# leaner-forever/SEGS-SLAM

Hardware: AMD Instinct MI355X
Metric: mapper train-iters/sec (fwd+bwd raster) (higher is better)
Workload: dtype f32; 1 GPU; 1080p_3m: 3000000 Gaussians, 1920x1080, 1 keyframe per GPU, fwd+bwd raster; P=3000000, P_visible=2096178, num_rendered=10472370, instances_binned=7913347, instances_live=6766534, width=1920, height=1080, parallelism=keyframe-dp1, forward=resident (no host sync), hipgraph=off

## Files before the change

include/segs_raster.h:

```cpp
#ifndef SEGS_RASTER_H_
#define SEGS_RASTER_H_

#include <stddef.h>
#include <stdint.h>

#ifdef __cplusplus
extern "C" {
#endif

#define SEGS_OK 0
#define SEGS_ERR_INVALID_ARGUMENT (-1)
#define SEGS_ERR_UNSUPPORTED (-2)
#define SEGS_ERR_ALLOC (-3)

typedef char* (*segs_alloc_fn)(void* ctx, size_t bytes);

const char* segs_last_error(void);

#define SEGS_RASTER_SKIP_NONPOSITIVE_OPACITY 1u
#define SEGS_RASTER_KEEP_DEAD_INSTANCES 2u
#define SEGS_RASTER_GATHER_TILES_TOUCHED 4u
#define SEGS_RASTER_TEST_NARROW_PACK 8u
#define SEGS_RASTER_UNFUSED_BINNING 16u
#define SEGS_RASTER_TIGHT_BINNING 32u
#define SEGS_RASTER_MFMA_MOMENTS 64u
#define SEGS_RASTER_NO_WRITTEN_BYTES 128u
uint32_t segs_raster_set_flags(uint32_t flags);

uint32_t* segs_raster_set_status_mirror(uint32_t* host_mapped_status);

size_t segs_geometry_bytes(int P);
size_t segs_image_bytes(int width, int height);
size_t segs_binning_bytes(int num_rendered);

int segs_rasterize_forward(segs_alloc_fn geometry_alloc, void* geometry_ctx,
                           segs_alloc_fn binning_alloc, void* binning_ctx,
                           segs_alloc_fn image_alloc, void* image_ctx,
                           int P, int D, int M,
                           const float* background, int width, int height,
                           const float* means3D, const float* shs, const float* colors_precomp,
                           const float* opacities, const float* scales, float scale_modifier,
                           const float* rotations, const float* cov3D_precomp,
                           const float* viewmatrix, const float* projmatrix, const float* cam_pos,
                           float tan_fovx, float tan_fovy, int prefiltered,
                           float* out_color, int* radii, void* stream, int* num_rendered);

int segs_rasterize_backward(int P, int D, int M, int R,
                            const float* background, int width, int height,
                            const float* means3D, const float* shs, const float* colors_precomp,
                            const float* scales, float scale_modifier, const float* rotations,
                            const float* cov3D_precomp, const float* viewmatrix, const float* projmatrix,
                            const float* campos, float tan_fovx, float tan_fovy, const int* radii,
                            char* geom_buffer, char* binning_buffer, char* image_buffer,
                            const float* dL_dpix, float* dL_dmean2D, float* dL_dconic, float* dL_dopacity,
                            float* dL_dcolor, float* dL_dmean3D, float* dL_dcov3D, float* dL_dsh,
                            float* dL_dscale, float* dL_drot, void* stream);

int segs_visible_filter(int P, int M, int width, int height, const float* means3D, const float* scales,
                        float scale_modifier, const float* rotations, const float* cov3D_precomp,
                        const float* viewmatrix, const float* projmatrix, float tan_fovx, float tan_fovy,
                        int prefiltered, int* radii, void* stream);

int segs_visible_filter_log_scales(int P, int width, int height, const float* means3D, const float* scaling_log, int stride,
                                   const float* rotations, const float* viewmatrix, const float* projmatrix, float tan_fovx,
                                   float tan_fovy, int* radii, void* stream);

int segs_mark_visible(int P, const float* means3D, const float* viewmatrix, const float* projmatrix,
                      uint8_t* present, void* stream);

int segs_project2_image(int P, int D, int M, int width, int height, const float* means3D, const float* shs,
                        const float* colors_precomp, const float* opacities, const float* scales,
                        float scale_modifier, const float* rotations, const float* cov3D_precomp,
                        const float* viewmatrix, const float* projmatrix, const float* cam_pos,
                        float tan_fovx, float tan_fovy, int prefiltered, float* out_color, float* points_image,
                        int* radii, void* stream);

int segs_debug_unpack_geometry(const char* geom_buffer, int P, const int* radii, float* means2D ,
                               float* conic_opacity , float* depths , uint32_t* tiles_touched ,
                               uint32_t* point_offsets , float* rgb , void* stream);
// ... 147 lines not shown
```

segs-slam_amd/csrc/capi.hip:

```cpp
#include <hip/hip_runtime.h>
#include <cstdio>
#include <cstdlib>
#include <algorithm>
#include <cstring>
#include <string>
#include <vector>
#include "../../include/segs_raster.h"
#include "gs_layout.h"
#include "kernels.h"
#include "capi_args.h"

using namespace segs;

namespace {
thread_local std::string g_err;
}
int segs::set_error(int code, const char* what) {
  g_err = what;
  return code;
}
int segs::set_hip_error(hipError_t e, const char* where) {
  g_err = std::string(where) + ": " + hipGetErrorString(e);
  return (int)e > 0 ? (int)e : 1;
}
// ... 238 lines not shown
  PROF(K_RENDER_FWD);
  if (dout && (dout->depth || dout->alpha))
    render_fwd_depth_kernel<<<V.tiles, 256, 0, st>>>(S.ranges(), S.point_list(), V.width, V.height, S.G.rec(), background, S.final_T(),
                                                     S.n_contrib(), out_color, dout->depth, dout->alpha);
  else
    render_fwd_kernel<<<V.tiles, 256, 0, st>>>(S.ranges(), S.point_list(), V.width, V.height, S.G.rec(), background, S.final_T(), S.n_contrib(),
                                               out_color);
  LAUNCH_TRY("render_fwd_kernel");
  return SEGS_OK;
}

int launch_render_bwd(const Scratch& S, const View& V, const float* background, const float* dL_dpix, const segs_depth_grads* dgrad,
                      uint8_t* written, hipStream_t st) {
  PROF(K_RENDER_BWD);
  const uint32_t grid = (V.tiles + 7) / 8 * 32;
  if (dgrad && (dgrad->dL_ddepth || dgrad->dL_dalpha)) {
    render_bwd_depth_kernel<<<grid, 64, 0, st>>>(S.ranges(), S.point_list(), V.width, V.height, S.G.rec(), background, S.final_T(),
                                                 S.n_contrib(), dL_dpix, S.G.gacc(), V.tiles, dgrad->dL_ddepth, dgrad->dL_dalpha, written);
    LAUNCH_TRY("render_bwd_depth_kernel");
    return SEGS_OK;
  }
  static const bool mfma_env = [] { const char* e = getenv("SEGS_RENDER_BWD_MFMA"); return e && e[0] == '1'; }();
  ((mfma_env || (g_flags & SEGS_RASTER_MFMA_MOMENTS)) ? render_bwd_mfma_kernel : render_bwd_kernel)<<<grid, 64, 0, st>>>(
      S.ranges(), S.point_list(), V.width, V.height, S.G.rec(), background, S.final_T(), S.n_contrib(), dL_dpix, S.G.gacc(), V.tiles, written);
  LAUNCH_TRY("render_bwd_kernel");
  return SEGS_OK;
}

int camera_grads_begin(const segs_camera_grads* cam, const float* shs, bool empty, hipStream_t st, bool* live) {
  *live = false;
  if (!cam) return SEGS_OK;
  if (!cam->dL_dviewmatrix || !cam->dL_dprojmatrix || !cam->temp) return fail(SEGS_ERR_INVALID_ARGUMENT, "segs_camera_grads: null field");
  if (shs) return fail(SEGS_ERR_INVALID_ARGUMENT, "camera gradients need colors_precomp: the SH colours depend on campos, which they do not cover");
  if (empty) {
    HIP_TRY(hipMemsetAsync(cam->dL_dviewmatrix, 0, 16 * sizeof(float), st));
    HIP_TRY(hipMemsetAsync(cam->dL_dprojmatrix, 0, 16 * sizeof(float), st));
    return SEGS_OK;
  }
  *live = true;
  return SEGS_OK;
}
float* camera_partials(const segs_camera_grads* cam) { return (float*)align_ptr(cam->temp); }
int camera_grads_finish(const segs_camera_grads* cam, int nblocks, hipStream_t st) {
  camera_grad_reduce_kernel<<<1, 960, 0, st>>>(camera_partials(cam), nblocks, cam->dL_dviewmatrix, cam->dL_dprojmatrix);
  LAUNCH_TRY("camera_grad_reduce_kernel");
  return SEGS_OK;
}

int launch_preprocess_bwd(const Gaussians& g, const View& V, const int* radii, const GradOutputs& o, const PerGaussianBwd& m, hipStream_t st) {
  const bool depth = m.depth || m.dz_in;
  auto* const kernel = m.cam ? (depth ? preprocess_bwd_kernel<true, true> : preprocess_bwd_kernel<false, true>)
                             : (depth ? preprocess_bwd_kernel<true, false> : preprocess_bwd_kernel<false, false>);
  const int nblocks = (g.P + 255) / 256;
  kernel<<<nblocks, 256, 0, st>>>(g.P, g.means3D, radii, g.kernel_scales(), g.rotations, g.scale_modifier, g.cov3D_precomp, V.viewmatrix,
                                  V.projmatrix, V.focal_x, V.focal_y, V.tan_fovx, V.tan_fovy, m.gacc, (float)V.width, (float)V.height,
                                  o.dL_dmean2D, o.dL_dconic, o.dL_dopacity, o.dL_dcolor, o.dL_dmean3D, o.dL_dcov3D, o.dL_dscale, o.dL_drot,
                                  m.clean_gacc ? 1 : 0, m.dz_in, m.cam ? camera_partials(m.cam) : nullptr, m.written);
  LAUNCH_TRY("preprocess_bwd_kernel");
  return m.cam ? camera_grads_finish(m.cam, nblocks, st) : SEGS_OK;
}

int rasterize_forward(const Allocators& A, const Gaussians& g, const View& V, const float* background, float* out_color, int* radii,
                      const segs_depth_outputs* dout, hipStream_t st, int* num_rendered) {
  const int P = g.P;
  if (!A.geometry_alloc || !A.binning_alloc || !A.image_alloc) return fail(SEGS_ERR_INVALID_ARGUMENT, "null allocator callback");
  if (P < 0 || V.width <= 0 || V.height <= 0) return fail(SEGS_ERR_INVALID_ARGUMENT, "bad P / image size");
  if (P > MAX_GAUSSIANS) return fail(SEGS_ERR_INVALID_ARGUMENT, "P exceeds 2^28 Gaussians (sort values carry a 4-bit quadrant mask)");
  if (!background || !out_color || !V.viewmatrix || !V.projmatrix || !num_rendered) return fail(SEGS_ERR_INVALID_ARGUMENT, "null required pointer");
  if (P > 0 && (!g.means3D || !g.opacities)) return fail(SEGS_ERR_INVALID_ARGUMENT, "null means3D/opacities");
  if (P > 0)
    if (int rc = check_colour_and_shape(g, V)) return rc;
  if (int rc = check_tile_grid(V)) return rc;

  Scratch S{};
  char* geom_raw = A.geometry_alloc(A.geometry_ctx, geom_layout(P).total);
  S.IL = image_layout(V.width, V.height);
  char* img_raw = A.image_alloc(A.image_ctx, S.IL.total);
  if (!geom_raw || !img_raw) return fail(SEGS_ERR_ALLOC, "allocator callback returned null");
  S.G = geom_at(geom_raw, P);
  S.img = align_ptr(img_raw);
  const Geom& G = S.G;
  if (!radii) radii = G.radii_internal();

  int R = 0;
  uint32_t hdr[3] = {0u, 0u, 0u};
  const bool tight = (g_flags & SEGS_RASTER_TIGHT_BINNING) != 0u;
  bool fast_keys = tight;
  if (P > 0) {
    K1Targets k1;
    k1.extra_flags = tight ? PREPROCESS_TIGHT_RECT : 0u;
    if (fast_keys) { k1.depth_keys = (uint32_t*)G.bin(); k1.ranges = S.ranges(); }
    int rc = run_preprocess(G, g, V, radii, k1, st);
    if (rc) return rc;
    { PROF(K_SCAN);
    scan_block_sums_kernel<<<1, 1024, 0, st>>>(G.block_sums(), G.L.nblocks, G.block_sums() + (G.L.nblocks + 1), G.num_rendered());
    }
    LAUNCH_TRY("scan_block_sums_kernel");
    HIP_TRY(hipMemcpyAsync(hdr, G.num_rendered(), sizeof(hdr), hipMemcpyDeviceToHost, st));
    HIP_TRY(hipStreamSynchronize(st));
    R = (int)hdr[0];
    if (R < 0) return fail(SEGS_ERR_INVALID_ARGUMENT, "num_rendered overflows int32");
    if (fast_keys && R > 0 && (hdr[2] - DEPTH_KEY_MIN) >= ((1u << DEPTH_KEY_BITS) - 1u)) {
      fast_keys = false;
      K1Targets exact;
      exact.extra_flags = PREPROCESS_TIGHT_RECT;
      rc = run_preprocess(G, g, V, radii, exact, st);
// ... 26 lines not shown
  if (B.geom_rows > MAX_GAUSSIANS) return fail(SEGS_ERR_INVALID_ARGUMENT, "P exceeds 2^28 Gaussians");
  if (!B.geom_buffer || !B.binning_buffer || !B.image_buffer || !status || !others_present) return fail(SEGS_ERR_INVALID_ARGUMENT, "null required pointer");
  if (k1)
    if (int rc = check_colour_and_shape(*k1, V)) return rc;
  if (int rc = check_tile_grid(V)) return rc;
  *S = carve(B, P, V, status);
  return SEGS_OK;
}

int rasterize_forward_resident(const ScratchBuffers& B, int P, const Gaussians* k1, const View& V, const float* background, float* out_color,
                               int* radii, uint32_t* status, const segs_depth_outputs* dout, hipStream_t st) {
  Scratch S{};
  const bool others_present = background && out_color && (!k1 || (V.viewmatrix && V.projmatrix && k1->means3D && k1->opacities));
  if (int rc = open_resident(B, P, V, status, others_present, k1, &S)) return rc;
  const DepthSortInput keys = resident_depth_sort_input(S.bin, S.GS);
  if (k1) {
    K1Targets t;
    t.depth_keys = keys.keys; t.depth_vals = keys.vals; t.ranges = S.ranges();
    t.extra_flags = resident_k1_flags(); t.depth_overflow = status + 2;
    if (int rc = run_preprocess(S.G, *k1, V, radii ? radii : S.G.radii_internal(), t, st)) return rc;
  }
  if (int rc = run_binning(S, V, BinningMode::resident_keys(keys.keys, drop_dead_instances()), st)) return rc;
  return launch_render_fwd(S, V, background, out_color, dout, st);
}

int rasterize_backward(const Gaussians& g, const View& V, const ScratchBuffers& B, const BackwardInputs& in, const GradOutputs& o,
                       GaccCleaning cleaning, hipStream_t st) {
  const int P = g.P, R = B.capacity;
  const bool self_clean = cleaning == SELF_CLEAN;
  if (P < 0 || R < 0 || V.width <= 0 || V.height <= 0) return fail(SEGS_ERR_INVALID_ARGUMENT, "bad sizes");
  if (B.geom_rows < P) return fail(SEGS_ERR_INVALID_ARGUMENT, "geom_rows must be >= P");
  bool cam_live = false;
  if (int rc = camera_grads_begin(in.cam, g.shs, P == 0 || R == 0, st, &cam_live)) return rc;
  if (P == 0) return SEGS_OK;
  if (g.shs && (!V.cam_pos || !o.dL_dsh || g.M <= 0)) return fail(SEGS_ERR_INVALID_ARGUMENT, "SH path needs campos, dL_dsh and M > 0");
  if (!B.geom_buffer || !B.binning_buffer || !B.image_buffer || !in.dL_dpix || !in.background || !g.means3D || !V.viewmatrix || !V.projmatrix)
    return fail(SEGS_ERR_INVALID_ARGUMENT, "null required pointer");
  if (!o.dL_dmean2D || !o.dL_dopacity || !o.dL_dcolor || !o.dL_dmean3D || (g.cov3D_precomp && !o.dL_dcov3D))
    return fail(SEGS_ERR_INVALID_ARGUMENT, "null gradient output");
  if (!g.cov3D_precomp && (!g.scales || !g.rotations || !o.dL_dscale || !o.dL_drot))
    return fail(SEGS_ERR_INVALID_ARGUMENT, "need scales+rotations (+ their gradient outputs) or cov3D_precomp");
  uint32_t* const no_status = nullptr;
  const Scratch S = carve(B, P, V, no_status);
  const Geom& G = S.G;
  const int* radii = in.radii ? in.radii : G.radii_internal();

  if (!self_clean) { PROF(K_MEMSET);
  HIP_TRY(hipMemsetAsync(G.gacc(), 0, (size_t)P * GACC_DWORDS * 4, st));
  }
  PerGaussianBwd m;
  m.gacc = G.gacc(); m.depth = in.dgrad && in.dgrad->dL_ddepth; m.clean_gacc = self_clean;
  if (cam_live) m.cam = in.cam;
  m.written = (self_clean && !(g_flags & SEGS_RASTER_NO_WRITTEN_BYTES)) ? G.written() : nullptr;
  if (R > 0)
    if (int rc = launch_render_bwd(S, V, in.background, in.dL_dpix, in.dgrad, m.written, st)) return rc;
  { PROF(K_PREPROCESS_BWD);
  if (int rc = launch_preprocess_bwd(g, V, radii, o, m, st)) return rc;
  }
  if (g.shs) {
    sh_backward_kernel<<<G.L.nblocks, 256, 0, st>>>(P, g.means3D, radii, g.shs, g.D, g.M, V.cam_pos, G.clamped(), o.dL_dcolor, o.dL_dmean3D, o.dL_dsh);
    LAUNCH_TRY("sh_backward_kernel");
  }
  return SEGS_OK;
}

int visible_filter(const Gaussians& g, const View& V, int log_scale_stride, int* radii, hipStream_t st) {
  if (g.P < 0 || V.width <= 0 || V.height <= 0) return fail(SEGS_ERR_INVALID_ARGUMENT, "bad sizes");
  if (g.P == 0) return SEGS_OK;
  if (!g.means3D || !V.viewmatrix || !V.projmatrix || !radii) return fail(SEGS_ERR_INVALID_ARGUMENT, "null required pointer");
  if (!g.cov3D_precomp && (!g.scales || !g.rotations)) return fail(SEGS_ERR_INVALID_ARGUMENT, "need scales+rotations or cov3D_precomp");
  visible_filter_kernel<<<(g.P + 255) / 256, 256, 0, st>>>(g.P, g.means3D, g.kernel_scales(), g.scale_modifier, g.rotations, g.cov3D_precomp,
                                                           V.viewmatrix, V.projmatrix, V.width, V.height, V.tan_fovx, V.tan_fovy, V.focal_x,
                                                           V.focal_y, V.gx, V.gy, radii, log_scale_stride);
  LAUNCH_TRY("visible_filter_kernel");
  return SEGS_OK;
}

int debug_preprocess_backward(const Gaussians& g, const View& V, const int* radii, const GradOutputs& o, const float* dL_dz,
                              const segs_camera_grads* cam, hipStream_t st) {
  bool cam_live = false;
  if (int rc = camera_grads_begin(cam, g.shs, g.P <= 0, st, &cam_live)) return rc;
  if (g.P <= 0) return SEGS_OK;
  if (!g.means3D || !radii || !V.viewmatrix || !V.projmatrix || !o.dL_dmean2D || !o.dL_dconic || !o.dL_dmean3D || !o.dL_dcov3D)
    return fail(SEGS_ERR_INVALID_ARGUMENT, "null pointer");
  PerGaussianBwd m;
  if (cam_live) { m.dz_in = dL_dz; m.cam = cam; }
  return launch_preprocess_bwd(g, V, radii, o, m, st);
}

}

extern "C" {

const char* segs_last_error(void) { return g_err.c_str(); }

uint32_t* segs_raster_set_status_mirror(uint32_t* host_mapped_status) {
  uint32_t* old = g_status_mirror;
  g_status_mirror = host_mapped_status;
  return old;
}

uint32_t segs_raster_set_flags(uint32_t flags) {
  const uint32_t old = g_flags;
  g_flags = flags;
  return old;
}
// ... 395 lines not shown
```

segs-slam_amd/csrc/capi_args.h:

```cpp
#pragma once
#include <hip/hip_runtime.h>
#include <cstdint>
#include "../../include/segs_raster.h"
#include "gs_layout.h"
#include "kernels.h"

namespace segs {

struct Gaussians {
  int P; const float *means3D, *scales; float scale_modifier; const float *rotations, *cov3D_precomp;
  int D, M; const float *shs, *colors_precomp, *opacities;
  const float* kernel_scales() const { return cov3D_precomp ? nullptr : scales; }
};

struct View {
  int width, height; const float *viewmatrix, *projmatrix, *cam_pos; float tan_fovx, tan_fovy;
  uint32_t gx, gy, tiles; float focal_x, focal_y;
};
inline View image_view(int width, int height) {
  View v{};
  v.width = width; v.height = height;
  v.gx = (width + TILE_X - 1) / TILE_X; v.gy = (height + TILE_Y - 1) / TILE_Y; v.tiles = v.gx * v.gy;
  return v;
}
// ... 54 lines not shown
  ImageLayout IL;
  BinningLayout BL;
  GaussSortLayout GS;
  uint32_t* status;
  uint2* ranges() const { return (uint2*)(img + IL.ranges); }
  const uint32_t* point_list() const { return (const uint32_t*)(bin + BL.vals[0]); }
  float* final_T() const { return (float*)(img + IL.final_T); }
  uint32_t* n_contrib() const { return (uint32_t*)(img + IL.n_contrib); }
};
inline Scratch carve(const ScratchBuffers& B, int P, const View& V, uint32_t* status) {
  return Scratch{geom_at(B.geom_buffer, P, B.geom_rows), align_ptr(B.image_buffer), align_ptr(B.binning_buffer), image_layout(V.width, V.height),
                 binning_layout(B.capacity), gauss_sort_layout(B.capacity, P), status};
}

struct DepthSortInput { uint32_t *keys, *vals; };
inline DepthSortInput depth_sort_input(char* bin, const GaussSortLayout& GS, int dbits, int digit_bits) {
  const int side = sort_first_side(dbits, digit_bits);
  return DepthSortInput{(uint32_t*)(bin + GS.base + GS.inner.keys[side]), (uint32_t*)(bin + GS.base + GS.inner.vals[side])};
}

struct BinningMode {
  uint32_t dmin; int dbits; uint32_t dcull;
  int digit_bits;
  const uint32_t* k1_keys;
  bool drop_dead;
  static constexpr int RESIDENT_DIGIT_BITS = 9;
  static BinningMode resident_keys(const uint32_t* k1_keys, bool drop_dead) {
    return BinningMode{DEPTH_KEY_MIN, DEPTH_KEY_BITS, 0xFFFFFFFFu, RESIDENT_DIGIT_BITS, k1_keys, drop_dead};
  }
  static BinningMode exact_range(uint32_t max_not_depth, uint32_t max_depth, bool drop_dead) {
    const uint32_t dmin = ~max_not_depth, dspan = max_depth - dmin + 1u;
    int dbits = 1;
    while (dbits < 32 && (dspan >> dbits) != 0u) dbits++;
    const bool nine = (dbits + 8) / 9 < (dbits + 7) / 8;
    return BinningMode{dmin, dbits, dmin + dspan, nine ? 9 : 8, nullptr, drop_dead};
  }
};
inline DepthSortInput resident_depth_sort_input(char* bin, const GaussSortLayout& GS) { return depth_sort_input(bin, GS, DEPTH_KEY_BITS, BinningMode::RESIDENT_DIGIT_BITS); }

struct K1Targets {
  uint32_t *depth_keys = nullptr, *depth_vals = nullptr;
  uint2* ranges = nullptr;
  uint32_t extra_flags = 0u;
  uint32_t* depth_overflow = nullptr;
};

struct PerGaussianBwd {
  float* gacc = nullptr;
  bool depth = false;
  bool clean_gacc = false;
  const float* dz_in = nullptr;
  const segs_camera_grads* cam = nullptr;
  uint8_t* written = nullptr;
};

struct Allocators { segs_alloc_fn geometry_alloc; void* geometry_ctx; segs_alloc_fn binning_alloc; void* binning_ctx; segs_alloc_fn image_alloc; void* image_ctx; };

enum GaccCleaning { MEMSET_PER_CALL, SELF_CLEAN };
struct BackwardInputs { const float* background; const int* radii; const float* dL_dpix; const segs_depth_grads* dgrad; const segs_camera_grads* cam; };

constexpr const Gaussians* K1_RAN_AT_PRODUCER = nullptr;
constexpr const segs_depth_outputs* NO_DEPTH_OUTPUTS = nullptr;
constexpr const segs_depth_grads* NO_DEPTH_GRADS = nullptr;
constexpr const segs_camera_grads* NO_CAMERA_GRADS = nullptr;
constexpr const float *NO_CAM_POS = nullptr, *NO_DL_DZ = nullptr;
constexpr int* NO_RADII = nullptr;

}
```

segs-slam_amd/csrc/kernels.h:

```cpp
#pragma once
#include <hip/hip_runtime.h>
#include <cstdint>
#include "gs_layout.h"

namespace segs {

int set_error(int code, const char* what);
int set_hip_error(hipError_t e, const char* where);


__global__ void preprocess_fwd_kernel(
    int P, const float* __restrict__ means3D, const float* __restrict__ scales, float mod,
    const float* __restrict__ rotations, const float* __restrict__ opacities, const float* __restrict__ colors,
    const float* __restrict__ cov3D_precomp, const float* __restrict__ viewmatrix, const float* __restrict__ projmatrix,
    int W, int H, float tan_fovx, float tan_fovy, float focal_x, float focal_y, uint32_t gx, uint32_t gy,
    int* __restrict__ radii, float* __restrict__ rec, BinInfo* __restrict__ bin, uint32_t* __restrict__ block_sums,
    uint32_t* __restrict__ depth_range, const float* __restrict__ shs, int D, int M, const float* __restrict__ cam_pos,
    uint32_t* __restrict__ clamped, uint32_t flags, uint32_t* __restrict__ depth_keys, uint32_t* __restrict__ depth_vals,
    uint2* __restrict__ ranges, int num_tiles, uint32_t* __restrict__ depth_overflow, uint32_t* __restrict__ touched_dense);
constexpr uint32_t DEPTH_KEY_MIN = 0x3E4CCCCDu;
constexpr int DEPTH_KEY_BITS = 27;

__global__ void visible_filter_kernel(
    int P, const float* __restrict__ means3D, const float* __restrict__ scales, float mod,
    const float* __restrict__ rotations, const float* __restrict__ cov3D_precomp,
    const float* __restrict__ viewmatrix, const float* __restrict__ projmatrix, int W, int H,
    float tan_fovx, float tan_fovy, float focal_x, float focal_y, uint32_t gx, uint32_t gy, int* __restrict__ radii,
    int log_scale_stride);

__global__ void mark_visible_kernel(int P, const float* __restrict__ means3D, const float* __restrict__ viewmatrix,
                                    uint8_t* __restrict__ present);

constexpr int CAM_SUMS = 24;
template <bool DEPTH, bool CAM>
__global__ void preprocess_bwd_kernel(
    int P, const float* __restrict__ means3D, const int* __restrict__ radii, const float* __restrict__ scales,
    const float* __restrict__ rotations, float mod, const float* __restrict__ cov3D_precomp,
    const float* __restrict__ view, const float* __restrict__ proj, float h_x, float h_y, float tan_fovx, float tan_fovy,
    float* __restrict__ gacc, float img_w, float img_h,
    float* __restrict__ dL_dmean2D, float* __restrict__ dL_dconic,
    float* __restrict__ dL_dopacity, float* __restrict__ dL_dcolor, float* __restrict__ dL_dmean3D,
    float* __restrict__ dL_dcov3D, float* __restrict__ dL_dscale, float* __restrict__ dL_drot, int clean_gacc,
    const float* __restrict__ dz_in, float* __restrict__ cam_partials, uint8_t* __restrict__ written);
__global__ void camera_grad_reduce_kernel(const float* __restrict__ partials, int nblocks, float* __restrict__ dL_dview,
                                          float* __restrict__ dL_dproj);
__global__ void sh_backward_kernel(int P, const float* __restrict__ means3D, const int* __restrict__ radii,
                                   const float* __restrict__ shs, int D, int M, const float* __restrict__ cam_pos,
                                   const uint32_t* __restrict__ clamped, const float* __restrict__ dL_dcolor,
                                   float* __restrict__ dL_dmean3D, float* __restrict__ dL_dsh);

__global__ void scan_block_sums_kernel(uint32_t* __restrict__ block_sums, int nblocks, const uint32_t* __restrict__ depth_range,
                                       uint32_t* __restrict__ total);
__global__ void ordered_offsets_kernel(int P, const uint32_t* __restrict__ block_sums, uint32_t* __restrict__ incl,
                                       uint32_t* __restrict__ total_out, const uint32_t* __restrict__ ng_dev,
                                       uint32_t* __restrict__ first_owner, uint32_t owner_entries);
__global__ void duplicate_with_keys_kernel(int P, int R, const float* __restrict__ rec,
                                           const uint32_t* __restrict__ order, const uint32_t* __restrict__ incl,
                                           uint32_t* __restrict__ keys, uint32_t* __restrict__ vals, uint32_t gx,
                                           const uint32_t* __restrict__ n_dev, int mark_dead, const uint32_t* __restrict__ ng_dev,
                                           const uint32_t* __restrict__ first_owner);
constexpr uint32_t RANGE_EMPTY_START = 0xFFFFFFFFu;
__global__ void normalize_ranges_kernel(int num_tiles, uint2* __restrict__ ranges);
constexpr uint32_t PREPROCESS_TIGHT_RECT = 0x80000000u;
constexpr uint32_t DEAD_KEY = 0xFFFFFFFFu;
template <typename K, int BITS>
__global__ void radix_count_kernel(const K* __restrict__ keys, int n, int shift, uint32_t dmin, int dbits,
                                   uint32_t* __restrict__ tile_prefix, uint32_t* __restrict__ chunk_hist, int nblocks, int nchunks,
                                   const uint32_t* __restrict__ n_dev, int drop_dead, int chunk_tiles, int nbits);
__global__ void radix_scan_kernel(uint32_t* __restrict__ block_hist, int nblocks, uint32_t* __restrict__ digit_totals);
template <typename K, int BITS, bool AUX>
__global__ void radix_scatter_kernel(const K* __restrict__ keys_in, const uint32_t* __restrict__ vals_in,
                                     K* __restrict__ keys_out, uint32_t* __restrict__ vals_out, int n, int shift,
                                     uint32_t dmin, int dbits, const uint32_t* __restrict__ tile_prefix, const uint32_t* __restrict__ chunk_prefix,
                                     const uint32_t* __restrict__ digit_totals, int nblocks, int nchunks,
                                     const uint32_t* __restrict__ n_dev, int drop_dead, uint32_t* __restrict__ n_live_out,
                                     const uint32_t* __restrict__ aux_in, uint32_t* __restrict__ aux_out, int nbits, int chunk_tiles, int pack_shift,
                                     uint2* __restrict__ ranges_out, uint32_t* __restrict__ status, uint32_t* __restrict__ status_mirror,
                                     int write_keys);
__global__ void identify_tile_ranges_kernel(int L, const uint32_t* __restrict__ keys, uint2* __restrict__ ranges,
                                            const uint32_t* __restrict__ n_dev, uint32_t* __restrict__ status,
                                            uint32_t* __restrict__ status_mirror, const uint32_t* __restrict__ n_live);

__global__ void render_fwd_kernel(const uint2* __restrict__ ranges, const uint32_t* __restrict__ point_list, int W, int H,
                                  const float* __restrict__ rec, const float* __restrict__ bg,
                                  float* __restrict__ final_T, uint32_t* __restrict__ n_contrib, float* __restrict__ out_color);
__global__ void render_bwd_kernel(const uint2* __restrict__ ranges, const uint32_t* __restrict__ point_list, int W, int H,
                                  const float* __restrict__ rec, const float* __restrict__ bg,
                                  const float* __restrict__ final_T, const uint32_t* __restrict__ n_contrib,
                                  const float* __restrict__ dL_dpix, float* __restrict__ gacc, uint32_t num_tiles,
                                  uint8_t* __restrict__ written);
__global__ void render_bwd_mfma_kernel(const uint2* __restrict__ ranges, const uint32_t* __restrict__ point_list, int W, int H,
                                       const float* __restrict__ rec, const float* __restrict__ bg,
                                       const float* __restrict__ final_T, const uint32_t* __restrict__ n_contrib,
                                       const float* __restrict__ dL_dpix, float* __restrict__ gacc, uint32_t num_tiles,
                                       uint8_t* __restrict__ written);
__global__ void render_fwd_depth_kernel(const uint2* __restrict__ ranges, const uint32_t* __restrict__ point_list, int W, int H,
// ... 27 lines not shown
```

segs-slam_amd/csrc/preprocess.hip:

```cpp
#include <hip/hip_runtime.h>
#include <cstdint>
#include "gs_layout.h"
#include "kernels.h"
#include "project_gaussian.h"
#include "sh_color.h"

#pragma clang fp contract(off)

namespace segs {

__device__ __forceinline__ float3 load_row3(const float* __restrict__ a, int P, float* lds ) {
  const int tid = threadIdx.x;
  const size_t base = (size_t)blockIdx.x * 768;
  const size_t lim = (size_t)P * 3;
#pragma unroll
  for (int k = 0; k < 3; k++) {
    const size_t i = base + k * 256 + tid;
    lds[k * 256 + tid] = i < lim ? a[i] : 0.f;
  }
  __syncthreads();
  float3 v = make_float3(lds[3 * tid], lds[3 * tid + 1], lds[3 * tid + 2]);
  __syncthreads();
  return v;
}
// ... 381 lines not shown
      for (int kk = 0; kk < 3; kk++) {
        float ds = 0.f;
#pragma unroll
        for (int i = 0; i < 3; i++) {
          const float dLik = 2.f * (M2[0][i] * DU[0][kk] + M2[1][i] * DU[1][kk]);
          ds += R[i][kk] * dLik;
          GR[i][kk] = dLik * s3[kk];
        }
        out_scale[kk] = ds;
      }
      const float r = q.x, x = q.y, y = q.z, z = q.w;
      out_rot[0] = 2.f * (z * (GR[1][0] - GR[0][1]) + y * (GR[0][2] - GR[2][0]) + x * (GR[2][1] - GR[1][2]));
      out_rot[1] = 2.f * (y * (GR[0][1] + GR[1][0]) + z * (GR[0][2] + GR[2][0]) + r * (GR[2][1] - GR[1][2])) - 4.f * x * (GR[1][1] + GR[2][2]);
      out_rot[2] = 2.f * (x * (GR[0][1] + GR[1][0]) + r * (GR[0][2] - GR[2][0]) + z * (GR[1][2] + GR[2][1])) - 4.f * y * (GR[0][0] + GR[2][2]);
      out_rot[3] = 2.f * (r * (GR[1][0] - GR[0][1]) + x * (GR[0][2] + GR[2][0]) + y * (GR[1][2] + GR[2][1])) - 4.f * z * (GR[0][0] + GR[1][1]);
    }
  }
  if constexpr (CAM) {
    const int v = threadIdx.x >> 5, l = threadIdx.x & 31;
#pragma unroll
    for (int pass = 0; pass < CAM_SUMS / 8; pass++) {
#pragma unroll
      for (int k = 0; k < 8; k++) lds[k * 256 + threadIdx.x] = cam[pass * 8 + k];
      __syncthreads();
      float s = lds[v * 256 + l];
#pragma unroll
      for (int q = 1; q < 8; q++) s += lds[v * 256 + l + 32 * q];
#pragma unroll
      for (int off = 16; off > 0; off >>= 1) s += __shfl_down(s, off, 64);
      if (l == 0) cam_partials[(size_t)blockIdx.x * CAM_SUMS + pass * 8 + v] = s;
      __syncthreads();
    }
  }
  if (gacc) store_row3(dL_dmean2D, P, lds, g2x, g2y, 0.f);
  store_row3(dL_dmean3D, P, lds, out_mean[0], out_mean[1], out_mean[2]);
  if (dL_dscale) store_row3(dL_dscale, P, lds, out_scale[0], out_scale[1], out_scale[2]);
  if (!live) return;
  if (dL_dcov3D) {
#pragma unroll
    for (int e = 0; e < 6; e++) dL_dcov3D[6 * (size_t)idx + e] = out_cov[e];
  }
  if (dL_drot) reinterpret_cast<float4*>(dL_drot)[idx] = make_float4(out_rot[0], out_rot[1], out_rot[2], out_rot[3]);
}

#define SEGS_PREPROCESS_BWD_ARGS int, const float*, const int*, const float*, const float*, float, const float*, const float*, \
    const float*, float, float, float, float, float*, float, float, float*, float*, float*, float*, float*, float*, float*, float*, int, \
    const float*, float*, uint8_t*
template __global__ void preprocess_bwd_kernel<false, false>(SEGS_PREPROCESS_BWD_ARGS);
template __global__ void preprocess_bwd_kernel<true, false>(SEGS_PREPROCESS_BWD_ARGS);
template __global__ void preprocess_bwd_kernel<false, true>(SEGS_PREPROCESS_BWD_ARGS);
template __global__ void preprocess_bwd_kernel<true, true>(SEGS_PREPROCESS_BWD_ARGS);
#undef SEGS_PREPROCESS_BWD_ARGS

__global__ void __launch_bounds__(960) camera_grad_reduce_kernel(const float* __restrict__ partials, int nblocks,
                                                                 float* __restrict__ dL_dview, float* __restrict__ dL_dproj) {
  __shared__ float rows[160 * CAM_SUMS];
  __shared__ float mid[10 * CAM_SUMS];
  __shared__ float sums[CAM_SUMS];
  const int t = threadIdx.x, q = t % 6, r0 = t / 6;
  float4 acc = make_float4(0.f, 0.f, 0.f, 0.f);
#pragma unroll 8
  for (int r = r0; r < nblocks; r += 160) {
    const float4 x = reinterpret_cast<const float4*>(partials + (size_t)r * CAM_SUMS)[q];
    acc.x += x.x; acc.y += x.y; acc.z += x.z; acc.w += x.w;
  }
  reinterpret_cast<float4*>(rows + r0 * CAM_SUMS)[q] = acc;
  __syncthreads();
  if (t < 10 * CAM_SUMS) {
    const int v = t % CAM_SUMS, g = t / CAM_SUMS;
    float s = 0.f;
    for (int k = 0; k < 16; k++) s += rows[(16 * g + k) * CAM_SUMS + v];
    mid[g * CAM_SUMS + v] = s;
  }
  __syncthreads();
  if (t < CAM_SUMS) {
    float s = 0.f;
    for (int g = 0; g < 10; g++) s += mid[g * CAM_SUMS + t];
    sums[t] = s;
  }
  __syncthreads();
  if (t < 32) {
    const int e = t & 15, i = e & 3, j = e >> 2;
    if (t < 16) dL_dview[e] = i < 3 ? sums[3 * j + i] : 0.f;
    else dL_dproj[e] = i != 2 ? sums[12 + 3 * j + (i == 3 ? 2 : i)] : 0.f;
  }
}

__global__ void __launch_bounds__(256) sh_backward_kernel(int P, const float* __restrict__ means3D, const int* __restrict__ radii,
                                                          const float* __restrict__ shs, int D, int M, const float* __restrict__ cam_pos,
                                                          const uint32_t* __restrict__ clamped, const float* __restrict__ dL_dcolor,
                                                          float* __restrict__ dL_dmean3D, float* __restrict__ dL_dsh) {
  const int idx = blockIdx.x * 256 + threadIdx.x;
  if (idx >= P || radii[idx] <= 0) return;
  const float3 mean = make_float3(means3D[3 * (size_t)idx], means3D[3 * (size_t)idx + 1], means3D[3 * (size_t)idx + 2]);
  const float3 dcol = make_float3(dL_dcolor[3 * (size_t)idx], dL_dcolor[3 * (size_t)idx + 1], dL_dcolor[3 * (size_t)idx + 2]);
  const float3 g = sh::backward(idx, D, M, mean, cam_pos, shs, clamped[idx], dcol, dL_dsh);
  dL_dmean3D[3 * (size_t)idx] += g.x; dL_dmean3D[3 * (size_t)idx + 1] += g.y; dL_dmean3D[3 * (size_t)idx + 2] += g.z;
}

}
```

Baseline: 1032 iters/s.

## Add packed preprocess backward that compacts reached Gaussians into one wave

```diff
diff --git a/include/segs_raster.h b/include/segs_raster.h
--- a/include/segs_raster.h
+++ b/include/segs_raster.h
@@ -25,6 +25,7 @@
 #define SEGS_RASTER_TIGHT_BINNING 32u
 #define SEGS_RASTER_MFMA_MOMENTS 64u
 #define SEGS_RASTER_NO_WRITTEN_BYTES 128u
+#define SEGS_RASTER_UNPACKED_BACKWARD 256u
 uint32_t segs_raster_set_flags(uint32_t flags);
 
 uint32_t* segs_raster_set_status_mirror(uint32_t* host_mapped_status);
diff --git a/segs-slam_amd/csrc/capi.hip b/segs-slam_amd/csrc/capi.hip
--- a/segs-slam_amd/csrc/capi.hip
+++ b/segs-slam_amd/csrc/capi.hip
@@ -314,6 +314,16 @@
   auto* const kernel = m.cam ? (depth ? preprocess_bwd_kernel<true, true> : preprocess_bwd_kernel<false, true>)
                              : (depth ? preprocess_bwd_kernel<true, false> : preprocess_bwd_kernel<false, false>);
   const int nblocks = (g.P + 255) / 256;
+  if (m.packed) {
+    auto* const packed = m.cam ? (depth ? preprocess_bwd_packed_kernel<true, true> : preprocess_bwd_packed_kernel<false, true>)
+                               : (depth ? preprocess_bwd_packed_kernel<true, false> : preprocess_bwd_packed_kernel<false, false>);
+    packed<<<nblocks, 256, 0, st>>>(g.P, g.means3D, radii, g.kernel_scales(), g.rotations, g.scale_modifier, g.cov3D_precomp, V.viewmatrix,
+                                    V.projmatrix, V.focal_x, V.focal_y, V.tan_fovx, V.tan_fovy, m.gacc, (float)V.width, (float)V.height,
+                                    o.dL_dmean2D, o.dL_dconic, o.dL_dopacity, o.dL_dcolor, o.dL_dmean3D, o.dL_dcov3D, o.dL_dscale, o.dL_drot,
+                                    m.cam ? camera_partials(m.cam) : nullptr, m.written);
+    LAUNCH_TRY("preprocess_bwd_packed_kernel");
+    return m.cam ? camera_grads_finish(m.cam, nblocks, st) : SEGS_OK;
+  }
   kernel<<<nblocks, 256, 0, st>>>(g.P, g.means3D, radii, g.kernel_scales(), g.rotations, g.scale_modifier, g.cov3D_precomp, V.viewmatrix,
                                   V.projmatrix, V.focal_x, V.focal_y, V.tan_fovx, V.tan_fovy, m.gacc, (float)V.width, (float)V.height,
                                   o.dL_dmean2D, o.dL_dconic, o.dL_dopacity, o.dL_dcolor, o.dL_dmean3D, o.dL_dcov3D, o.dL_dscale, o.dL_drot,
@@ -446,6 +456,7 @@
   m.gacc = G.gacc(); m.depth = in.dgrad && in.dgrad->dL_ddepth; m.clean_gacc = self_clean;
   if (cam_live) m.cam = in.cam;
   m.written = (self_clean && !(g_flags & SEGS_RASTER_NO_WRITTEN_BYTES)) ? G.written() : nullptr;
+  m.packed = m.written && !(g_flags & SEGS_RASTER_UNPACKED_BACKWARD);
   if (R > 0)
     if (int rc = launch_render_bwd(S, V, in.background, in.dL_dpix, in.dgrad, m.written, st)) return rc;
   { PROF(K_PREPROCESS_BWD);
diff --git a/segs-slam_amd/csrc/capi_args.h b/segs-slam_amd/csrc/capi_args.h
--- a/segs-slam_amd/csrc/capi_args.h
+++ b/segs-slam_amd/csrc/capi_args.h
@@ -130,6 +130,7 @@
   const float* dz_in = nullptr;
   const segs_camera_grads* cam = nullptr;
   uint8_t* written = nullptr;
+  bool packed = false;
 };
 
 struct Allocators { segs_alloc_fn geometry_alloc; void* geometry_ctx; segs_alloc_fn binning_alloc; void* binning_ctx; segs_alloc_fn image_alloc; void* image_ctx; };
diff --git a/segs-slam_amd/csrc/kernels.h b/segs-slam_amd/csrc/kernels.h
--- a/segs-slam_amd/csrc/kernels.h
+++ b/segs-slam_amd/csrc/kernels.h
@@ -42,6 +42,16 @@
     float* __restrict__ dL_dopacity, float* __restrict__ dL_dcolor, float* __restrict__ dL_dmean3D,
     float* __restrict__ dL_dcov3D, float* __restrict__ dL_dscale, float* __restrict__ dL_drot, int clean_gacc,
     const float* __restrict__ dz_in, float* __restrict__ cam_partials, uint8_t* __restrict__ written);
+template <bool DEPTH, bool CAM>
+__global__ void preprocess_bwd_packed_kernel(
+    int P, const float* __restrict__ means3D, const int* __restrict__ radii, const float* __restrict__ scales,
+    const float* __restrict__ rotations, float mod, const float* __restrict__ cov3D_precomp,
+    const float* __restrict__ view, const float* __restrict__ proj, float h_x, float h_y, float tan_fovx, float tan_fovy,
+    float* __restrict__ gacc, float img_w, float img_h,
+    float* __restrict__ dL_dmean2D, float* __restrict__ dL_dconic,
+    float* __restrict__ dL_dopacity, float* __restrict__ dL_dcolor, float* __restrict__ dL_dmean3D,
+    float* __restrict__ dL_dcov3D, float* __restrict__ dL_dscale, float* __restrict__ dL_drot,
+    float* __restrict__ cam_partials, uint8_t* __restrict__ written);
 __global__ void camera_grad_reduce_kernel(const float* __restrict__ partials, int nblocks, float* __restrict__ dL_dview,
                                           float* __restrict__ dL_dproj);
 __global__ void sh_backward_kernel(int P, const float* __restrict__ means3D, const int* __restrict__ radii,
diff --git a/segs-slam_amd/csrc/preprocess.hip b/segs-slam_amd/csrc/preprocess.hip
--- a/segs-slam_amd/csrc/preprocess.hip
+++ b/segs-slam_amd/csrc/preprocess.hip
@@ -457,6 +457,354 @@
 template __global__ void preprocess_bwd_kernel<true, true>(SEGS_PREPROCESS_BWD_ARGS);
 #undef SEGS_PREPROCESS_BWD_ARGS
 
+template <bool DEPTH, bool CAM>
+__device__ __forceinline__ void projection_backward_row(
+    size_t idx, float3 mean, float3 scale, float4 q, float mod, const float* __restrict__ cov3D_precomp, bool has_scales, bool want_cov,
+    const float* __restrict__ view, const float* __restrict__ proj, float h_x, float h_y, float tan_fovx, float tan_fovy,
+    float img_w, float img_h, float4 a0, Sym2 G, float dz, float& g2x, float& g2y, float (&out_mean)[3], float (&out_cov)[6],
+    float (&out_scale)[3], float (&out_rot)[4], float (&cam)[CAM ? CAM_SUMS : 1]) {
+  const float tx0 = view[0] * mean.x + view[4] * mean.y + view[8] * mean.z + view[12];
+  const float ty0 = view[1] * mean.x + view[5] * mean.y + view[9] * mean.z + view[13];
+  const float tz = view[2] * mean.x + view[6] * mean.y + view[10] * mean.z + view[14];
+  const float limx = 1.3f * tan_fovx, limy = 1.3f * tan_fovy;
+  const float rx = tx0 / tz, ry = ty0 / tz;
+  const bool free_x = !(rx < -limx || rx > limx), free_y = !(ry < -limy || ry > limy);
+  const float tx = fminf(limx, fmaxf(-limx, rx)) * tz, ty = fminf(limy, fmaxf(-limy, ry)) * tz;
+  const float iz = 1.f / tz, iz2 = iz * iz;
+  const float J00 = h_x * iz, J02 = -h_x * tx * iz2, J11 = h_y * iz, J12 = -h_y * ty * iz2;
+  float M2[2][3];
+#pragma unroll
+  for (int j = 0; j < 3; j++) {
+    M2[0][j] = J00 * view[4 * j] + J02 * view[4 * j + 2];
+    M2[1][j] = J11 * view[4 * j + 1] + J12 * view[4 * j + 2];
+  }
+  float R[3][3] = {{0, 0, 0}, {0, 0, 0}, {0, 0, 0}}, s3[3] = {0, 0, 0};
+  float E[2][3];
+  float U[2][3] = {{0, 0, 0}, {0, 0, 0}};
+  float a, b, c;
+  if (cov3D_precomp) {
+    const float* cv = cov3D_precomp + (size_t)6 * idx;
+    const float S[3][3] = {{cv[0], cv[1], cv[2]}, {cv[1], cv[3], cv[4]}, {cv[2], cv[4], cv[5]}};
+#pragma unroll
+    for (int r = 0; r < 2; r++)
+#pragma unroll
+      for (int j = 0; j < 3; j++) E[r][j] = M2[r][0] * S[0][j] + M2[r][1] * S[1][j] + M2[r][2] * S[2][j];
+    a = E[0][0] * M2[0][0] + E[0][1] * M2[0][1] + E[0][2] * M2[0][2] + 0.3f;
+    b = E[0][0] * M2[1][0] + E[0][1] * M2[1][1] + E[0][2] * M2[1][2];
+    c = E[1][0] * M2[1][0] + E[1][1] * M2[1][1] + E[1][2] * M2[1][2] + 0.3f;
+    q = make_float4(0, 0, 0, 0);
+  } else {
+    quat_rows(q, R);
+    s3[0] = mod * scale.x; s3[1] = mod * scale.y; s3[2] = mod * scale.z;
+#pragma unroll
+    for (int r = 0; r < 2; r++)
+#pragma unroll
+      for (int k = 0; k < 3; k++) U[r][k] = (M2[r][0] * R[0][k] + M2[r][1] * R[1][k] + M2[r][2] * R[2][k]) * s3[k];
+#pragma unroll
+    for (int r = 0; r < 2; r++)
+#pragma unroll
+      for (int j = 0; j < 3; j++) E[r][j] = U[r][0] * R[j][0] * s3[0] + U[r][1] * R[j][1] * s3[1] + U[r][2] * R[j][2] * s3[2];
+    a = U[0][0] * U[0][0] + U[0][1] * U[0][1] + U[0][2] * U[0][2] + 0.3f;
+    b = U[0][0] * U[1][0] + U[0][1] * U[1][1] + U[0][2] * U[1][2];
+    c = U[1][0] * U[1][0] + U[1][1] * U[1][1] + U[1][2] * U[1][2] + 0.3f;
+  }
+  const float det = a * c - b * b;
+  const float k = 1.0f / (det * det + 0.0000001f);
+  {
+    const float di = 1.0f / det;
+    const float cA = c * di, cB = -b * di, cC = a * di;
+    g2x = -(cA * a0.x + cB * a0.y) * (0.5f * img_w);
+    g2y = -(cC * a0.y + cB * a0.x) * (0.5f * img_h);
+  }
+  const float h0 = c * G.xx - b * G.xy, h1 = c * G.xy - b * G.yy;
+  const float h2 = a * G.xy - b * G.xx, h3 = a * G.yy - b * G.xy;
+  Sym2 Dc;
+  Dc.xx = -k * (h0 * c - h1 * b);
+  Dc.xy = -k * (h1 * a - h0 * b);
+  Dc.yy = -k * (h3 * a - h2 * b);
+  float DM[2][3];
+#pragma unroll
+  for (int j = 0; j < 3; j++) { DM[0][j] = Dc.xx * M2[0][j] + Dc.xy * M2[1][j]; DM[1][j] = Dc.xy * M2[0][j] + Dc.yy * M2[1][j]; }
+  if (want_cov || cov3D_precomp) {
+    const int ii[6] = {0, 0, 0, 1, 1, 2}, jj[6] = {0, 1, 2, 1, 2, 2};
+#pragma unroll
+    for (int e = 0; e < 6; e++) {
+      const float v = M2[0][ii[e]] * DM[0][jj[e]] + M2[1][ii[e]] * DM[1][jj[e]];
+      out_cov[e] = ii[e] == jj[e] ? v : 2.f * v;
+    }
+  }
+  float dM2[2][3];
+#pragma unroll
+  for (int j = 0; j < 3; j++) {
+    dM2[0][j] = 2.f * (Dc.xx * E[0][j] + Dc.xy * E[1][j]);
+    dM2[1][j] = 2.f * (Dc.xy * E[0][j] + Dc.yy * E[1][j]);
+  }
+  const float dJ00 = dM2[0][0] * view[0] + dM2[0][1] * view[4] + dM2[0][2] * view[8];
+  const float dJ02 = dM2[0][0] * view[2] + dM2[0][1] * view[6] + dM2[0][2] * view[10];
+  const float dJ11 = dM2[1][0] * view[1] + dM2[1][1] * view[5] + dM2[1][2] * view[9];
+  const float dJ12 = dM2[1][0] * view[2] + dM2[1][1] * view[6] + dM2[1][2] * view[10];
+  const float iz3 = iz2 * iz;
+  const float dtx = free_x ? -h_x * iz2 * dJ02 : 0.f;
+  const float dty = free_y ? -h_y * iz2 * dJ12 : 0.f;
+  const float dtz = -h_x * iz2 * dJ00 - h_y * iz2 * dJ11 + 2.f * h_x * tx * iz3 * dJ02 + 2.f * h_y * ty * iz3 * dJ12;
+  const float hx = proj[0] * mean.x + proj[4] * mean.y + proj[8] * mean.z + proj[12];
+  const float hy = proj[1] * mean.x + proj[5] * mean.y + proj[9] * mean.z + proj[13];
+  const float hw = proj[3] * mean.x + proj[7] * mean.y + proj[11] * mean.z + proj[15];
+  const float w = 1.0f / (hw + 0.0000001f);
+  const float ux = hx * w * w, uy = hy * w * w;
+#pragma unroll
+  for (int j = 0; j < 3; j++) {
+    const float from_cov = view[4 * j] * dtx + view[4 * j + 1] * dty + view[4 * j + 2] * dtz;
+    const float from_proj = (proj[4 * j] * w - proj[4 * j + 3] * ux) * g2x + (proj[4 * j + 1] * w - proj[4 * j + 3] * uy) * g2y;
+    out_mean[j] = from_cov + from_proj;
+  }
+  if (DEPTH) {
+#pragma unroll
+    for (int j = 0; j < 3; j++) out_mean[j] += dz * view[4 * j + 2];
+  }
+  if constexpr (CAM) {
+    const float dtz_all = DEPTH ? dtz + dz : dtz;
+    const float pm[3] = {mean.x, mean.y, mean.z};
+    const float dh0 = g2x * w, dh1 = g2y * w, dh3 = -(g2x * hx + g2y * hy) * (w * w);
+#pragma unroll
+    for (int j = 0; j < 3; j++) {
+      cam[3 * j + 0] = dtx * pm[j] + J00 * dM2[0][j];
+      cam[3 * j + 1] = dty * pm[j] + J11 * dM2[1][j];
+      cam[3 * j + 2] = dtz_all * pm[j] + (J02 * dM2[0][j] + J12 * dM2[1][j]);
+      cam[12 + 3 * j + 0] = dh0 * pm[j];
+      cam[12 + 3 * j + 1] = dh1 * pm[j];
+      cam[12 + 3 * j + 2] = dh3 * pm[j];
+    }
+    cam[9] = dtx; cam[10] = dty; cam[11] = dtz_all;
+    cam[21] = dh0; cam[22] = dh1; cam[23] = dh3;
+  }
+  if (has_scales) {
+    float DU[2][3];
+#pragma unroll
+    for (int kk = 0; kk < 3; kk++) { DU[0][kk] = Dc.xx * U[0][kk] + Dc.xy * U[1][kk]; DU[1][kk] = Dc.xy * U[0][kk] + Dc.yy * U[1][kk]; }
+    float GR[3][3];
+#pragma unroll
+    for (int kk = 0; kk < 3; kk++) {
+      float ds = 0.f;
+#pragma unroll
+      for (int i = 0; i < 3; i++) {
+        const float dLik = 2.f * (M2[0][i] * DU[0][kk] + M2[1][i] * DU[1][kk]);
+        ds += R[i][kk] * dLik;
+        GR[i][kk] = dLik * s3[kk];
+      }
+      out_scale[kk] = ds;
+    }
+    const float r = q.x, x = q.y, y = q.z, z = q.w;
+    out_rot[0] = 2.f * (z * (GR[1][0] - GR[0][1]) + y * (GR[0][2] - GR[2][0]) + x * (GR[2][1] - GR[1][2]));
+    out_rot[1] = 2.f * (y * (GR[0][1] + GR[1][0]) + z * (GR[0][2] + GR[2][0]) + r * (GR[2][1] - GR[1][2])) - 4.f * x * (GR[1][1] + GR[2][2]);
+    out_rot[2] = 2.f * (x * (GR[0][1] + GR[1][0]) + r * (GR[0][2] - GR[2][0]) + z * (GR[1][2] + GR[2][1])) - 4.f * y * (GR[0][0] + GR[2][2]);
+    out_rot[3] = 2.f * (r * (GR[1][0] - GR[0][1]) + x * (GR[0][2] + GR[2][0]) + y * (GR[1][2] + GR[2][1])) - 4.f * z * (GR[0][0] + GR[1][1]);
+  }
+}
+
+template <int D>
+__device__ __forceinline__ void zero_window(float* __restrict__ a, size_t first, int rows, int zt, int nz,
+                                            const uint64_t* reached_masks ) {
+  if (!a) return;
+  float* const w = a + first * D;
+  const int lim = rows * D;
+  for (int i = zt; i < lim; i += nz) {
+    const int row = i / D;
+    if (!((reached_masks[row >> 6] >> (row & 63)) & 1ull)) w[i] = 0.f;
+  }
+}
+
+template <bool DEPTH, bool CAM>
+__global__ void __launch_bounds__(256) preprocess_bwd_packed_kernel(
+    int P, const float* __restrict__ means3D, const int* __restrict__ radii, const float* __restrict__ scales,
+    const float* __restrict__ rotations, float mod, const float* __restrict__ cov3D_precomp,
+    const float* __restrict__ view, const float* __restrict__ proj, float h_x, float h_y, float tan_fovx, float tan_fovy,
+    float* __restrict__ gacc, float img_w, float img_h,
+    float* __restrict__ dL_dmean2D, float* __restrict__ dL_dconic,
+    float* __restrict__ dL_dopacity, float* __restrict__ dL_dcolor, float* __restrict__ dL_dmean3D,
+    float* __restrict__ dL_dcov3D, float* __restrict__ dL_dscale, float* __restrict__ dL_drot,
+    float* __restrict__ cam_partials, uint8_t* __restrict__ written) {
+  __shared__ float lds[3 * 768];
+  __shared__ __attribute__((aligned(16))) float gl[4][32 * GACC_DWORDS];
+  __shared__ uint64_t wave_mask[4];
+  __shared__ uint16_t list[64];
+  const int tid = threadIdx.x, lane = tid & 63, wave = tid >> 6;
+  const size_t first = (size_t)blockIdx.x * 256;
+  const int rows = (size_t)P - first < 256 ? (int)((size_t)P - first) : 256;
+  const bool live = tid < rows;
+  const bool reached = live && written[first + tid] != 0;
+  const uint64_t mask = __ballot(reached);
+  if (lane == 0) wave_mask[wave] = mask;
+  __syncthreads();
+  const int c0 = __popcll(wave_mask[0]), c1 = __popcll(wave_mask[1]), c2 = __popcll(wave_mask[2]), c3 = __popcll(wave_mask[3]);
+  const int n = __builtin_amdgcn_readfirstlane(c0 + c1 + c2 + c3);
+  if (n > 0 && wave == 3 && lane * 4 < rows) reinterpret_cast<uint32_t*>(written + first)[lane] = 0u;
+
+  float g2x = 0.f, g2y = 0.f;
+  Sym2 G{0.f, 0.f, 0.f};
+  float dcol0 = 0.f, dcol1 = 0.f, dcol2 = 0.f, dop = 0.f, dz = 0.f;
+  float out_mean[3] = {0, 0, 0}, out_cov[6] = {0, 0, 0, 0, 0, 0}, out_scale[3] = {0, 0, 0}, out_rot[4] = {0, 0, 0, 0};
+  float cam[CAM ? CAM_SUMS : 1] = {0};
+  const int v = tid >> 5, l = tid & 31;
+
+  if (n > 64) {
+    const size_t idx = first + tid;
+    const bool binned = reached && radii[idx] > 0;
+    float3 mean, scale, unused;
+    load_rows3(means3D, scales, nullptr, P, lds, mean, scale, unused);
+    float4 a0 = make_float4(0.f, 0.f, 0.f, 0.f), a1 = a0;
+    {
+      float* const wl = gl[wave];
+      const size_t wave_first = first + (tid & ~63);
+#pragma unroll
+      for (int half = 0; half < 2; half++) {
+        float4 q[2];
+#pragma unroll
+        for (int j = 0; j < 2; j++) {
+          const int r = 16 * j + (lane >> 2), owner = 32 * half + r;
+          q[j] = make_float4(0.f, 0.f, 0.f, 0.f);
+          if (((mask >> owner) & 1ull) && (lane & 3) < 3) {
+            float4* src = reinterpret_cast<float4*>(gacc + (wave_first + owner) * GACC_DWORDS) + (lane & 3);
+            q[j] = *src;
+            *src = make_float4(0.f, 0.f, 0.f, 0.f);
+          }
+        }
+#pragma unroll
+        for (int j = 0; j < 2; j++) reinterpret_cast<float4*>(wl + (16 * j + (lane >> 2)) * GACC_DWORDS)[lane & 3] = q[j];
+        asm volatile("" ::: "memory");
+        if ((lane >> 5) == half) {
+          const float4* mine = reinterpret_cast<const float4*>(wl + (lane & 31) * GACC_DWORDS);
+          a0 = mine[0]; a1 = mine[1]; dcol2 = wl[(lane & 31) * GACC_DWORDS + 8];
+          if (DEPTH) dz = wl[(lane & 31) * GACC_DWORDS + 9];
+        }
+        asm volatile("" ::: "memory");
+      }
+    }
+    if (binned) {
+      G.xx = -0.5f * a0.z; G.xy = -0.5f * a0.w; G.yy = -0.5f * a1.x;
+      dop = a1.y;
+      dcol0 = a1.z; dcol1 = a1.w;
+    }
+    store_row3(dL_dcolor, P, lds, dcol0, dcol1, dcol2);
+    if (live) {
+      if (dL_dconic) reinterpret_cast<float4*>(dL_dconic)[idx] = make_float4(G.xx, G.xy, 0.f, G.yy);
+      dL_dopacity[idx] = dop;
+    }
+    if (binned) {
+      const float4 rot = cov3D_precomp ? make_float4(0, 0, 0, 0) : reinterpret_cast<const float4*>(rotations)[idx];
+      projection_backward_row<DEPTH, CAM>(idx, mean, scale, rot, mod, cov3D_precomp, scales != nullptr, dL_dcov3D != nullptr, view, proj, h_x,
+                                          h_y, tan_fovx, tan_fovy, img_w, img_h, a0, G, dz, g2x, g2y, out_mean, out_cov, out_scale, out_rot, cam);
+    }
+    if constexpr (CAM) {
+#pragma unroll
+      for (int pass = 0; pass < CAM_SUMS / 8; pass++) {
+#pragma unroll
+        for (int k = 0; k < 8; k++) lds[k * 256 + tid] = cam[pass * 8 + k];
+        __syncthreads();
+        float s = lds[v * 256 + l];
+#pragma unroll
+        for (int q = 1; q < 8; q++) s += lds[v * 256 + l + 32 * q];
+#pragma unroll
+        for (int off = 16; off > 0; off >>= 1) s += __shfl_down(s, off, 64);
+        if (l == 0) cam_partials[(size_t)blockIdx.x * CAM_SUMS + pass * 8 + v] = s;
+        __syncthreads();
+      }
+    }
+    store_row3(dL_dmean2D, P, lds, g2x, g2y, 0.f);
+    store_row3(dL_dmean3D, P, lds, out_mean[0], out_mean[1], out_mean[2]);
+    if (dL_dscale) store_row3(dL_dscale, P, lds, out_scale[0], out_scale[1], out_scale[2]);
+    if (!live) return;
+    if (dL_dcov3D) {
+#pragma unroll
+      for (int e = 0; e < 6; e++) dL_dcov3D[6 * idx + e] = out_cov[e];
+    }
+    if (dL_drot) reinterpret_cast<float4*>(dL_drot)[idx] = make_float4(out_rot[0], out_rot[1], out_rot[2], out_rot[3]);
+    return;
+  }
+
+  if (reached) list[(wave > 0 ? c0 : 0) + (wave > 1 ? c1 : 0) + (wave > 2 ? c2 : 0) + __popcll(mask & ((1ull << lane) - 1ull))] = (uint16_t)tid;
+  __syncthreads();
+  const bool heavy = wave == 0 && lane < n;
+  int r = 0;
+  size_t g = first;
+  if (wave == 0) {
+    int radius = 0;
+    float3 mean = make_float3(0, 0, 0), scale = mean;
+    float4 rot = make_float4(0, 0, 0, 0), a0 = rot, a1 = rot, a2 = rot;
+    if (heavy) {
+      r = list[lane];
+      g = first + r;
+      radius = radii[g];
+      mean = make_float3(means3D[3 * g], means3D[3 * g + 1], means3D[3 * g + 2]);
+      if (scales) scale = make_float3(scales[3 * g], scales[3 * g + 1], scales[3 * g + 2]);
+      if (!cov3D_precomp) rot = reinterpret_cast<const float4*>(rotations)[g];
+      float4* const src = reinterpret_cast<float4*>(gacc + g * GACC_DWORDS);
+      a0 = src[0]; a1 = src[1]; a2 = src[2];
+      const float4 z4 = make_float4(0.f, 0.f, 0.f, 0.f);
+      src[0] = z4; src[1] = z4; src[2] = z4;
+      dcol2 = a2.x;
+      if (DEPTH) dz = a2.y;
+    }
+    if (heavy && radius > 0) {
+      G.xx = -0.5f * a0.z; G.xy = -0.5f * a0.w; G.yy = -0.5f * a1.x;
+      dop = a1.y;
+      dcol0 = a1.z; dcol1 = a1.w;
+      projection_backward_row<DEPTH, CAM>(g, mean, scale, rot, mod, cov3D_precomp, scales != nullptr, dL_dcov3D != nullptr, view, proj, h_x, h_y,
+                                          tan_fovx, tan_fovy, img_w, img_h, a0, G, dz, g2x, g2y, out_mean, out_cov, out_scale, out_rot, cam);
+    }
+    if (heavy) {
+      dL_dcolor[3 * g] = dcol0; dL_dcolor[3 * g + 1] = dcol1; dL_dcolor[3 * g + 2] = dcol2;
+      if (dL_dconic) reinterpret_cast<float4*>(dL_dconic)[g] = make_float4(G.xx, G.xy, 0.f, G.yy);
+      dL_dopacity[g] = dop;
+      dL_dmean2D[3 * g] = g2x; dL_dmean2D[3 * g + 1] = g2y; dL_dmean2D[3 * g + 2] = 0.f;
+      dL_dmean3D[3 * g] = out_mean[0]; dL_dmean3D[3 * g + 1] = out_mean[1]; dL_dmean3D[3 * g + 2] = out_mean[2];
+      if (dL_dscale) { dL_dscale[3 * g] = out_scale[0]; dL_dscale[3 * g + 1] = out_scale[1]; dL_dscale[3 * g + 2] = out_scale[2]; }
+      if (dL_dcov3D) {
+#pragma unroll
+        for (int k = 0; k < 6; k++) dL_dcov3D[6 * g + k] = out_cov[k];
+      }
+      if (dL_drot) reinterpret_cast<float4*>(dL_drot)[g] = make_float4(out_rot[0], out_rot[1], out_rot[2], out_rot[3]);
+    }
+  } else {
+    const int zt = tid - 64, nz = 192;
+    zero_window<3>(dL_dcolor, first, rows, zt, nz, wave_mask);
+    zero_window<4>(dL_dconic, first, rows, zt, nz, wave_mask);
+    zero_window<1>(dL_dopacity, first, rows, zt, nz, wave_mask);
+    zero_window<3>(dL_dmean2D, first, rows, zt, nz, wave_mask);
+    zero_window<3>(dL_dmean3D, first, rows, zt, nz, wave_mask);
+    zero_window<3>(dL_dscale, first, rows, zt, nz, wave_mask);
+    zero_window<6>(dL_dcov3D, first, rows, zt, nz, wave_mask);
+    zero_window<4>(dL_drot, first, rows, zt, nz, wave_mask);
+  }
+  if constexpr (CAM) {
+#pragma unroll
+    for (int pass = 0; pass < CAM_SUMS / 8; pass++) {
+#pragma unroll
+      for (int k = 0; k < 8; k++) {
+        if (!reached) lds[k * 256 + tid] = 0.f;
+        if (heavy) lds[k * 256 + r] = cam[pass * 8 + k];
+      }
+      __syncthreads();
+      float s = lds[v * 256 + l];
+#pragma unroll
+      for (int q = 1; q < 8; q++) s += lds[v * 256 + l + 32 * q];
+#pragma unroll
+      for (int off = 16; off > 0; off >>= 1) s += __shfl_down(s, off, 64);
+      if (l == 0) cam_partials[(size_t)blockIdx.x * CAM_SUMS + pass * 8 + v] = s;
+      __syncthreads();
+    }
+  }
+}
+
+#define SEGS_PREPROCESS_BWD_PACKED_ARGS int, const float*, const int*, const float*, const float*, float, const float*, const float*, \
+    const float*, float, float, float, float, float*, float, float, float*, float*, float*, float*, float*, float*, float*, float*, \
+    float*, uint8_t*
+template __global__ void preprocess_bwd_packed_kernel<false, false>(SEGS_PREPROCESS_BWD_PACKED_ARGS);
+template __global__ void preprocess_bwd_packed_kernel<true, false>(SEGS_PREPROCESS_BWD_PACKED_ARGS);
+template __global__ void preprocess_bwd_packed_kernel<false, true>(SEGS_PREPROCESS_BWD_PACKED_ARGS);
+template __global__ void preprocess_bwd_packed_kernel<true, true>(SEGS_PREPROCESS_BWD_PACKED_ARGS);
+#undef SEGS_PREPROCESS_BWD_PACKED_ARGS
+
 __global__ void __launch_bounds__(960) camera_grad_reduce_kernel(const float* __restrict__ partials, int nblocks,
                                                                  float* __restrict__ dL_dview, float* __restrict__ dL_dproj) {
   __shared__ float rows[160 * CAM_SUMS];
```

Measured after the change: 1051 iters/s (median of 6 runs). 1.8% higher.
